# VojtaHavlicek/AlphaZero-Piskvorky

Measured on AMD Instinct MI355X. Metric: mcts_node_expansions_per_sec, higher is better.
Workload: dtype f32; 1 GPU; 15x15 / 5-in-a-row self-play, 1024 concurrent games per GPU, 400 sims/move (BASELINE.json configs[3] per-GPU shard), GomokuNet random-init weights, numpy-compatible RNG tapes; board=15, win_length=5, sims_per_move=400, games_per_gpu=1024, engines_per_gpu=4, search_kernel=lock-step (k_trunk, k_fc, k_step per evaluation batch), parallelism=games sharded x1

## Files before the change

alphazero-piskvorky_amd/_capi.py:

```python
import ctypes as C
import os
import subprocess

import numpy as np

_HERE = os.path.dirname(os.path.abspath(__file__))
LIB_PATH = os.environ.get("AZ_ENGINE_LIB") or os.path.join(_HERE, "libaz_engine.so")

STATE_DICT_ORDER = [
    "conv1.weight", "conv1.bias", "conv2.weight", "conv2.bias", "conv3.weight", "conv3.bias",
    "policy_conv.weight", "policy_conv.bias", "policy_fc.weight", "policy_fc.bias",
    "value_conv.weight", "value_conv.bias", "value_fc1.weight", "value_fc1.bias",
    "value_fc2.weight", "value_fc2.bias",
]

AZ_EVAL_NET, AZ_EVAL_SYNTHETIC = 0, 1
AZ_RES_NONE, AZ_RES_X, AZ_RES_O, AZ_RES_DRAW = 0, 1, 2, 3
AZ_AUG_NONE, AZ_AUG_REFERENCE4, AZ_AUG_DIHEDRAL8 = 1, 4, 8
AZ_MODEL_PLAIN, AZ_MODEL_RESNET = 0, 1
AZ_TRUNK_F32, AZ_TRUNK_BF16X3, AZ_TRUNK_F16X2 = 0, 1, 2
AZ_MAX_SIMULATIONS, AZ_DEEP_MAX_SIMULATIONS = 1024, 65534
REUSE_MAX_SIMULATIONS = 1023

EXPORTS = [
    "az_create", "az_create_deep", "az_destroy", "az_last_error", "az_load_weights", "az_load_weights_resnet", "az_net_eval", "az_search", "az_search_batch", "az_search_callback", "az_selfplay",
    "az_selfplay_begin", "az_selfplay_step", "az_selfplay_end", "az_selfplay_games", "az_selfplay_records", "az_selfplay_clear", "az_record_bytes", "az_selfplay_pack", "az_examples_from_packed",
    "az_examples_gather", "az_arena", "az_rules_replay", "az_rng_selfplay_tape", "az_rng_uniforms", "az_set_profiling", "az_set_subtree_reuse", "az_get_counters", "az_get_lanes", "az_get_persistent", "az_set_virtual_loss", "az_set_eval_cache",
    "az_set_trunk_mode", "az_get_trunk_mode", "az_set_leaf_symmetry", "az_emul_split",
    "az_set_start_positions", "az_get_start_positions",
    "az_set_resign", "az_get_resign", "az_selfplay_values", "az_selfplay_pack_values", "az_selfplay_resign_info",
    "az_resign_mix", "az_resign_exempt",
    "az_set_playout_cap", "az_get_playout_cap", "az_playout_cap_full", "az_selfplay_sims", "az_selfplay_export_count",
    "az_set_forced_playouts", "az_get_forced_playouts", "az_forced_prune",
    "az_set_selection", "az_get_selection", "az_selection_tables",
    "az_set_candidates", "az_get_candidates", "az_candidate_mask",
    "az_set_gumbel", "az_get_gumbel", "az_gumbel_schedule", "az_gumbel_target", "az_gumbel_vmix", "az_rng_selfplay_tape_gumbel",
    "az_set_external_evaluator", "az_get_external_evaluator", "az_ext_capacity", "az_ext_stats",
    "az_set_solver", "az_get_solver", "az_last_proof", "az_selfplay_proofs", "az_solver_counts", "az_solver_stops",
    "az_set_win_rule", "az_get_win_rule", "az_rules_winner",
    "az_set_threat_search", "az_get_threat_search", "az_threat_batch", "az_threat_solve", "az_selfplay_threats", "az_threat_stats",
    "az_set_rng", "az_get_rng", "az_rng_philox4x32", "az_rng_log", "az_rng_exp", "az_rng_philox_tape", "az_rng_philox_tape_device",
    "az_set_delta_eval", "az_get_delta_eval", "az_delta_max_tiles", "az_delta_stats", "az_net_eval_delta", "az_delta_lists",
    "az_dist_unique_id", "az_dist_init", "az_dist_rank", "az_dist_world", "az_dist_counts", "az_dist_gather_records",
    "az_dist_allreduce_sum", "az_dist_broadcast",
]
AZ_DIST_ID_BYTES = 128


class AzError(RuntimeError):
    pass


class az_config(C.Structure):
    _fields_ = [("board_size", C.c_int32), ("win_length", C.c_int32), ("num_simulations", C.c_int32),
                ("slots", C.c_int32), ("c_puct", C.c_double), ("dirichlet_alpha", C.c_double),
                ("dirichlet_weight", C.c_double), ("eval_kind", C.c_int32), ("device", C.c_int32),
                ("log_table", C.POINTER(C.c_float)), ("model", C.c_int32), ("engines", C.c_int32)]


class az_selfplay_args(C.Structure):
    _fields_ = [("seed0", C.c_uint64), ("num_games", C.c_int32), ("max_plies", C.c_int32),
                ("temperature_table", C.POINTER(C.c_double)), ("noise_tape", C.POINTER(C.c_double)),
                ("u_tape", C.POINTER(C.c_double)), ("tape_stride", C.c_int64)]


class az_counters(C.Structure):
    _fields_ = [("games", C.c_int64), ("plies", C.c_int64), ("records", C.c_int64), ("simulations", C.c_int64),
                ("expansions", C.c_int64), ("root_evals", C.c_int64), ("terminal_hits", C.c_int64),
                ("depth_sum", C.c_int64), ("steps", C.c_int64), ("seconds", C.c_double), ("nn_seconds", C.c_double),
                ("trunk_seconds", C.c_double), ("trunk_launches", C.c_int64), ("trunk_boards", C.c_int64),
                ("step_seconds", C.c_double), ("duplicate_leaves", C.c_int64), ("cache_lookups", C.c_int64),
                ("cache_hits", C.c_int64), ("tape_wait_seconds", C.c_double), ("tape_threads", C.c_int64),
                ("host_cpus", C.c_int64)]

    def as_dict(self):
        return {k: getattr(self, k) for k, _ in self._fields_}


class az_arena_args(C.Structure):
    _fields_ = [("seed0", C.c_uint64), ("num_games", C.c_int32), ("temperature_table", C.POINTER(C.c_double)),
                ("u_tape", C.POINTER(C.c_double))]


class az_arena_result(C.Structure):
    _fields_ = [("wins", C.c_int32), ("losses", C.c_int32), ("draws", C.c_int32), ("total", C.c_int32),
                ("win_rate", C.c_double)]


_EVAL_BATCH_FN = C.CFUNCTYPE(C.c_int, C.c_void_p, C.c_int, C.c_int)


class az_ext_evaluator(C.Structure):
    _fields_ = [("planes_dev", C.c_void_p), ("policy_dev", C.c_void_p), ("value_dev", C.c_void_p),
                ("capacity", C.c_int32), ("fn", _EVAL_BATCH_FN), ("user", C.c_void_p)]

# ... 62 lines not shown
            L.az_selfplay_export_count.argtypes = [C.c_void_p, C.POINTER(C.c_int64)]
        if hasattr(L, "az_set_forced_playouts"):
            L.az_set_forced_playouts.argtypes = [C.c_void_p, C.c_double, C.c_int]
            L.az_get_forced_playouts.argtypes = [C.c_void_p, C.POINTER(C.c_double), C.POINTER(C.c_int)]
            L.az_forced_prune.argtypes = [C.c_double, C.c_double, C.c_int, C.c_void_p, C.c_void_p, C.c_void_p, C.c_void_p]
            L.az_forced_prune.restype = C.c_int64
        if hasattr(L, "az_set_selection"):
            L.az_set_selection.argtypes = [C.c_void_p, C.c_int] + [C.c_double] * 4
            L.az_get_selection.argtypes = [C.c_void_p, C.POINTER(C.c_int)] + [C.POINTER(C.c_double)] * 4
            L.az_selection_tables.argtypes = [C.c_double, C.c_double, C.c_double, C.c_int, C.c_void_p, C.c_void_p]
        if hasattr(L, "az_set_candidates"):
            L.az_set_candidates.argtypes = [C.c_void_p, C.c_int]
            L.az_get_candidates.argtypes = [C.c_void_p, C.POINTER(C.c_int)]
            L.az_candidate_mask.argtypes = [C.c_int, C.c_void_p, C.c_int, C.c_void_p]
        if hasattr(L, "az_set_gumbel"):
            L.az_set_gumbel.argtypes = [C.c_void_p, C.c_int, C.c_double, C.c_double]
            L.az_get_gumbel.argtypes = [C.c_void_p, C.POINTER(C.c_int), C.POINTER(C.c_double), C.POINTER(C.c_double)]
            L.az_gumbel_schedule.argtypes = [C.c_int, C.c_int, C.c_void_p]
            L.az_gumbel_target.argtypes = [C.c_int, C.c_void_p, C.c_void_p, C.c_void_p, C.c_void_p, C.c_void_p, C.c_float, C.c_double,
                                           C.c_double, C.c_void_p, C.POINTER(C.c_int32)]
            L.az_gumbel_vmix.argtypes = [C.c_int, C.c_void_p, C.c_void_p, C.c_void_p, C.c_float]
            L.az_gumbel_vmix.restype = C.c_double
            L.az_rng_selfplay_tape_gumbel.argtypes = [C.c_uint64, C.c_int, C.c_int, C.c_void_p, C.c_void_p]
        if hasattr(L, "az_set_external_evaluator"):
            L.az_set_external_evaluator.argtypes = [C.c_void_p, C.POINTER(az_ext_evaluator)]
            L.az_get_external_evaluator.argtypes = [C.c_void_p]
            L.az_ext_capacity.argtypes = [C.c_void_p]
            L.az_ext_stats.argtypes = [C.c_void_p, C.POINTER(C.c_int64), C.POINTER(C.c_int64)]
        if hasattr(L, "az_set_solver"):
            L.az_set_solver.argtypes = [C.c_void_p, C.c_int]
            L.az_get_solver.argtypes = [C.c_void_p]
            L.az_last_proof.argtypes = [C.c_void_p, C.c_int, C.c_void_p, C.c_void_p, C.POINTER(C.c_int32)]
            L.az_solver_stops.argtypes = [C.c_void_p, C.POINTER(C.c_int64)]
            L.az_selfplay_proofs.argtypes = [C.c_void_p, C.c_void_p]
            L.az_solver_counts.argtypes = [C.c_int, C.c_void_p, C.c_void_p, C.c_void_p]
        if hasattr(L, "az_set_win_rule"):
            L.az_set_win_rule.argtypes = [C.c_void_p, C.c_int]
            L.az_get_win_rule.argtypes = [C.c_void_p]
            L.az_rules_winner.argtypes = [C.c_void_p, C.c_int, C.c_int, C.c_int]
        if hasattr(L, "az_set_threat_search"):
            L.az_set_threat_search.argtypes = [C.c_void_p, C.c_int, C.c_int]
            L.az_get_threat_search.argtypes = [C.c_void_p, C.POINTER(C.c_int), C.POINTER(C.c_int)]
            L.az_threat_batch.argtypes = [C.c_void_p, C.c_int, C.c_void_p, C.c_void_p, C.c_int, C.c_int] + [C.c_void_p] * 5
            L.az_threat_solve.argtypes = [C.c_void_p, C.c_int, C.c_int, C.c_int, C.c_int, C.c_int, C.c_int] + [C.c_void_p] * 4
            L.az_selfplay_threats.argtypes = [C.c_void_p, C.c_void_p]
            L.az_threat_stats.argtypes = [C.c_void_p] + [C.POINTER(C.c_int64)] * 5
        if hasattr(L, "az_set_delta_eval"):
            L.az_set_delta_eval.argtypes = [C.c_void_p, C.c_int]
            L.az_get_delta_eval.argtypes = [C.c_void_p]
            L.az_delta_max_tiles.argtypes = [C.c_void_p, C.c_int]
            L.az_delta_stats.argtypes = [C.c_void_p] + [C.POINTER(C.c_int64)] * 4 + [C.c_void_p]
            L.az_net_eval_delta.argtypes = [C.c_void_p, C.c_int, C.c_void_p, C.c_int, C.c_int] + [C.c_void_p] * 7
            L.az_delta_lists.argtypes = [C.c_int, C.c_int] + [C.c_void_p] * 5
        if hasattr(L, "az_set_rng"):
            L.az_set_rng.argtypes = [C.c_void_p, C.c_int]
            L.az_get_rng.argtypes = [C.c_void_p]
            L.az_rng_philox4x32.argtypes = [C.c_void_p, C.c_void_p, C.c_void_p]
            L.az_rng_philox4x32.restype = None
            L.az_rng_log.argtypes = L.az_rng_exp.argtypes = [C.c_double]
            L.az_rng_log.restype = L.az_rng_exp.restype = C.c_double
            L.az_rng_philox_tape.argtypes = [C.c_uint64, C.c_int, C.c_double, C.c_int, C.c_int, C.c_void_p, C.c_void_p]
            L.az_rng_philox_tape_device.argtypes = [C.c_void_p, C.c_uint64, C.c_int, C.c_double, C.c_int, C.c_int, C.c_void_p, C.c_void_p]
        _LIB = L
    return _LIB


def _p(a):
    return None if a is None else a.ctypes.data_as(C.c_void_p)


def _dp(a):
    return None if a is None else a.ctypes.data_as(C.POINTER(C.c_double))


def rng_selfplay_tape(seed, n, alpha=0.3, max_plies=0):
    nn = n * n
    plies = max_plies if 0 < max_plies < nn else nn
    total = sum(nn - m for m in range(plies))
    noise = np.zeros(total, np.float64)
    u = np.zeros(nn, np.float64)
    rc = lib().az_rng_selfplay_tape(int(seed), n, float(alpha), int(max_plies), _p(noise), _p(u))
    if rc:
        raise AzError(f"az_rng_selfplay_tape failed ({rc})")
    return noise, u[:plies]


def dist_unique_id():
    buf = C.create_string_buffer(AZ_DIST_ID_BYTES)
    rc = lib().az_dist_unique_id(buf)
    if rc:
        raise AzError(f"az_dist_unique_id failed ({rc}): {lib().az_last_error(None).decode()}")
    return buf.raw


def rng_uniforms(seed, count):
    u = np.zeros(count, np.float64)
    rc = lib().az_rng_uniforms(int(seed), int(count), _p(u))
    if rc:
        raise AzError(f"az_rng_uniforms failed ({rc})")
    return u


def resign_mix(key):
    return int(lib().az_resign_mix(int(key) & 0xFFFFFFFF))


# ... 845 lines not shown
```

alphazero-piskvorky_amd/csrc/az_delta.h:

```cpp
#pragma once
#include "az_net.h"

constexpr int DELTA_MAX_CHANGED = 8;
constexpr int DELTA_TILES_DEFAULT = 12;
constexpr int DELTA_CNT = 4 + 16;

template <int N>
struct DeltaGeo : NetGeo<N> {
    typedef NetGeo<N> B;
    static constexpr int IMG = 96 * B::CS;
    static constexpr int STRIDE = IMG + B::FROW;
    static constexpr int MAXM = ((B::nn + 15) / 16) * 16;
    static constexpr int C3 = 4;
};

__host__ __device__ inline int delta_dist(int n, int pr, int pc, const unsigned char *changed, int nch)
{
    int best = 255;
    for (int i = 0; i < nch; i++) {
        const int cr = changed[i] / n, cc = changed[i] - cr * n;
        const int dr = pr - 1 - cr < 0 ? cr - (pr - 1) : pr - 1 - cr, dc = pc - 1 - cc < 0 ? cc - (pc - 1) : pc - 1 - cc;
        const int dd = dr > dc ? dr : dc;
        best = dd < best ? dd : best;
    }
    return best;
}
__host__ __device__ inline bool delta_member(int n, int list, int pr, int pc, int dist)
{
    const bool inb = pr >= 1 && pr <= n && pc >= 1 && pc <= n;
    return list < 3 ? (inb && dist <= list + 1) : dist <= list;
}
template <int N>
struct DeltaLists {
    typedef DeltaGeo<N> G;
    unsigned short wpos[3][G::MAXM], cell[3][G::MAXM];
    unsigned short halo[2][G::PP];
    int cnt[5];
    __host__ __device__ int tiles(int l) const { return (cnt[l] + 15) >> 4; }
    __host__ __device__ void put(int list, int at, int pr, int pc)
    {
        const unsigned short pos = (unsigned short)(pr * G::PW + pc);
        if (list < 3) { wpos[list][at] = pos; cell[list][at] = (unsigned short)((pr - 1) * N + (pc - 1)); }
        else halo[list - 3][at] = pos;
    }
    __host__ __device__ void junk(int list, int i)
    {
        const int c = cnt[list], at = c + i;
        if (c > 0 && at < tiles(list) * 16) { wpos[list][at] = wpos[list][c - 1]; cell[list][at] = 0xFFFF; }
    }
};
template <int N>
__host__ __device__ inline void delta_lists_serial(const unsigned char *changed, int nch, DeltaLists<N> &L)
{
    typedef DeltaGeo<N> G;
    for (int l = 0; l < 5; l++) L.cnt[l] = 0;
    for (int p = 0; p < G::PP; p++) {
        const int pr = p / G::PW, pc = p - pr * G::PW;
        const int dist = delta_dist(N, pr, pc, changed, nch);
        for (int l = 0; l < 5; l++)
            if (delta_member(N, l, pr, pc, dist)) L.put(l, L.cnt[l]++, pr, pc);
    }
    for (int l = 0; l < 3; l++)
        for (int i = 0; i < 16; i++) L.junk(l, i);
}

#ifdef __HIPCC__
template <class G>
__device__ __forceinline__ void delta_heads(const NetWeights &w, float *__restrict__ frow, const float *out3, const float *hdq_lds,
                                            const unsigned short *cellof, int ncell, int wave, int lane)
{
    if (wave * 32 >= ncell) return;
    const int half = (lane >> 2) & 1;
    const int m = wave * 32 + (lane >> 3) * 4 + (lane & 3);
    float hb[4];
#pragma unroll
    for (int i = 0; i < 4; i++) hb[i] = (half * 4 + i) < 6 ? w.hdb[half * 4 + i] : 0.0f;
    const float4 *ap = reinterpret_cast<const float4 *>(hdq_lds) + (lane & 7);
    const float4 *bp = reinterpret_cast<const float4 *>(out3 + (m < ncell ? m : 0) * OUT3_CM_STRIDE);
    f32x4 acc = f32x4{0.f, 0.f, 0.f, 0.f};
#pragma unroll
    for (int k4 = 0; k4 < 32; k4++) {
        const float4 a = ap[k4 * 8], b = bp[k4];
        acc = __builtin_amdgcn_mfma_f32_4x4x1f32(a.x, b.x, acc, 0, 0, 0);
        acc = __builtin_amdgcn_mfma_f32_4x4x1f32(a.y, b.y, acc, 0, 0, 0);
        acc = __builtin_amdgcn_mfma_f32_4x4x1f32(a.z, b.z, acc, 0, 0, 0);
        acc = __builtin_amdgcn_mfma_f32_4x4x1f32(a.w, b.w, acc, 0, 0, 0);
    }
    if (m < ncell) {
        const int cell = cellof[m];
        if (cell != 0xFFFF) {
#pragma unroll
            for (int i = 0; i < 4; i++) {
                const int j = half * 4 + i;
                if (j < 6) {
                    float v = acc[i] + hb[i];
                    frow[j * G::nn + cell] = v > 0.0f ? v : 0.0f;
                }
            }
        }
    }
}

template <int N>
__global__ __launch_bounds__(NetGeo<N>::NW * 64) void k_trunk_base(DevState d, NetWeights w, int net_id, float *__restrict__ base,
                                                                    unsigned long long *cnt)
{
    typedef FusedGeo<N> G;
    typedef DeltaGeo<N> DG;
    static_assert(G::G == 1, "one board per workgroup");
    __shared__ __attribute__((aligned(16))) float lds[G::LDSF];
    __shared__ __attribute__((aligned(16))) float hdq_lds[1024];
    __shared__ unsigned short wpos[G::MR];
    __shared__ unsigned short cellof[G::MR];
    const int b = blockIdx.x, par = blockIdx.y;
    if (d.s_status[b] != SLOT_ACTIVE || d.s_net[b] != net_id) return;
    const int tid = threadIdx.x, lane = tid & 63;
    const int wave = __builtin_amdgcn_readfirstlane(tid >> 6);
    const float2 hq = reinterpret_cast<const float2 *>(w.hdq)[tid];
    bool e_me = false, e_op = false;
    int e_pos = G::PW + 1;
    if (tid < G::nn) {
        const int r = tid / N, c = tid - r * N;
        e_pos = (r + 1) * G::PW + (c + 1);
        const u64 *bd = d.board + (size_t)b * 8;
        const bool x = (bd[tid >> 6] >> (tid & 63)) & 1ull, o = (bd[4 + (tid >> 6)] >> (tid & 63)) & 1ull;
        const bool me_is_x = (d.s_player[b] == 1) != (par == 1);
        e_me = me_is_x ? x : o;
        e_op = me_is_x ? o : x;
    }
    reinterpret_cast<float2 *>(hdq_lds)[tid] = hq;
    if (tid < G::MR) {
        if constexpr (BorderSkip<G>::value) { wpos[tid] = G::map.pos[tid]; cellof[tid] = G::map.cell[tid]; }
        else {
            const int t = tid >> 4, c = tid & 15;
            wpos[tid] = (unsigned short)((t + 1) * G::PW + (c + 1));
            cellof[tid] = (unsigned short)(c < N ? t * N + c : 0xFFFF);
        }
    }
    {
        float4 *z = reinterpret_cast<float4 *>(lds);
        for (int i = tid; i < (96 * G::CS) / 4; i += G::NW * 64) z[i] = float4{0.f, 0.f, 0.f, 0.f};
    }
    __syncthreads();
    float *inA = lds, *inB = lds + 32 * G::CS;
    if (e_me) inB[e_pos] = 1.0f;
    if (e_op) inB[G::CS + e_pos] = 1.0f;
    __syncthreads();
    conv_layer<G, 4, 32, CONV_OUT_PACKED>(inB, inA, w.c1, w.c1b, wpos, cellof, wave, lane);
    __syncthreads();
    for (int i = tid; i < 3 * G::CS; i += G::NW * 64) inB[i] = 0.0f;
    __syncthreads();
    conv_layer<G, 32, 64, CONV_OUT_PACKED>(inA, inB, w.c2, w.c2b, wpos, cellof, wave, lane);
    __syncthreads();
    float *row = base + ((size_t)b * 2 + par) * DG::STRIDE;
    {
        const float4 *s = reinterpret_cast<const float4 *>(lds);
        float4 *g = reinterpret_cast<float4 *>(row);
        for (int i = tid; i < DG::IMG / 4; i += G::NW * 64) g[i] = s[i];
    }
    conv_layer<G, 64, 128, CONV_OUT3_CM>(inB, lds, w.c3, w.c3b, wpos, cellof, wave, lane);
    __syncthreads();
    trunk_heads<G>(d, w, net_id, row + DG::IMG - (size_t)b * G::FROW, lds, hdq_lds, cellof, b, wave, lane);
    if (tid == 0 && par == 0) cnt[(size_t)b * DELTA_CNT + 3] += 2ull;
}

template <int N>
__global__ __launch_bounds__(NetGeo<N>::NW * 64) void k_trunk_delta(DevState d, NetWeights w, int net_id, float *__restrict__ feat,
                                                                     const float *__restrict__ base, unsigned char *done,
                                                                     unsigned long long *cnt, int max_tiles)
{
    typedef DeltaGeo<N> G;
    constexpr int NT = G::NW * 64;
    static_assert(G::G == 1 && NT >= G::PP && NT == 512, "one board per workgroup, one thread per padded position");
    static_assert(G::C3 * 16 * OUT3_CM_STRIDE <= 32 * G::CS, "a chunk's conv3 image fits the dead conv1 image");
    static_assert(G::STRIDE % 4 == 0, "16-byte rows");
    __shared__ __attribute__((aligned(16))) float lds[G::IMG];
    __shared__ __attribute__((aligned(16))) float planes[4 * G::CS];
    __shared__ __attribute__((aligned(16))) float hdq_lds[1024];
    __shared__ DeltaLists<N> L;
    __shared__ unsigned char changed[DELTA_MAX_CHANGED];
    __shared__ unsigned char s_dist[G::PP];
    __shared__ int s_nch;
    __shared__ int s_wc[5][5];
    const int b = blockIdx.x;
    if (b >= d.B) return;
    const int tid = threadIdx.x, lane = tid & 63;
    const int wave = __builtin_amdgcn_readfirstlane(tid >> 6);
    {
        const int kind = d.leaf_kind[b];
        if (!((kind == LEAF_ROOT || kind == LEAF_EXPAND) && d.s_status[b] == SLOT_ACTIVE && d.s_net[b] == net_id)) {
            if (tid == 0) done[b] = 1;
            return;
        }
    }
    const float2 hq = reinterpret_cast<const float2 *>(w.hdq)[tid];
    const u64 *lf = d.leaf + (size_t)b * 8, *bd = d.board + (size_t)b * 8;
    const int last = d.leaf_last[b];
    int stones = 0;
#pragma unroll
    for (int i = 0; i < 8; i++) stones += __popcll(lf[i]) - __popcll(bd[i]);
    const int par = stones & 1;
    bool e_me = false, e_op = false, e_last = false;
    int e_pos = G::PW + 1;
    if (tid == 0) s_nch = 0;
    for (int i = tid; i < 4 * G::CS; i += NT) planes[i] = 0.0f;
    reinterpret_cast<float2 *>(hdq_lds)[tid] = hq;
    __syncthreads();
    if (tid < G::nn) {
        const int r = tid / N, c = tid - r * N;
        e_pos = (r + 1) * G::PW + (c + 1);
        e_me = (lf[tid >> 6] >> (tid & 63)) & 1ull;
        e_op = (lf[4 + (tid >> 6)] >> (tid & 63)) & 1ull;
        e_last = last == tid;
        const bool x = (bd[tid >> 6] >> (tid & 63)) & 1ull, o = (bd[4 + (tid >> 6)] >> (tid & 63)) & 1ull;
        const bool me_is_x = (d.s_player[b] == 1) != (par == 1);
        if (e_me != (me_is_x ? x : o) || e_op != (me_is_x ? o : x) || e_last) {
            const int k = atomicAdd(&s_nch, 1);
            if (k < DELTA_MAX_CHANGED) changed[k] = (unsigned char)tid;
        }
        if (e_me) planes[e_pos] = 1.0f;
        if (e_op) planes[G::CS + e_pos] = 1.0f;
        if (e_last) planes[2 * G::CS + e_pos] = 1.0f;
    }
    __syncthreads();
    const int nch = s_nch;
    if (nch > DELTA_MAX_CHANGED) {
        if (tid == 0) { done[b] = 0; cnt[(size_t)b * DELTA_CNT + 1] += 1ull; }
        return;
    }
    int dist = 255, pr = 0, pc = 0;
    u64 bal[5] = {0, 0, 0, 0, 0};
    if (wave < 5) {
        const bool in_img = tid < G::PP;
        if (in_img) {
            pr = tid / G::PW; pc = tid - pr * G::PW;
            dist = delta_dist(N, pr, pc, changed, nch);
            s_dist[tid] = (unsigned char)dist;
        }
#pragma unroll
        for (int l = 0; l < 5; l++) {
            bal[l] = __ballot(in_img && delta_member(N, l, pr, pc, dist));
            if (lane == 0) s_wc[wave][l] = __popcll(bal[l]);
        }
    }
    __syncthreads();
    if (wave < 5 && tid < G::PP) {
#pragma unroll
        for (int l = 0; l < 5; l++) {
            if (!((bal[l] >> lane) & 1ull)) continue;
            int at = __popcll(bal[l] & ((1ull << lane) - 1ull));
            for (int v = 0; v < wave; v++) at += s_wc[v][l];
            L.put(l, at, pr, pc);
        }
    }
    if (tid < 5) L.cnt[tid] = s_wc[0][tid] + s_wc[1][tid] + s_wc[2][tid] + s_wc[3][tid] + s_wc[4][tid];
    __syncthreads();
    const int t1 = L.tiles(0), t2 = L.tiles(1), t3 = L.tiles(2);
    if (t3 > max_tiles) {
        if (tid == 0) { done[b] = 0; cnt[(size_t)b * DELTA_CNT + 1] += 1ull; }
        return;
    }
    if (tid < 48) L.junk(tid >> 4, tid & 15);
    if (tid == 0) {
        done[b] = (unsigned char)(1 + t3);
        cnt[(size_t)b * DELTA_CNT + 0] += 1ull;
        cnt[(size_t)b * DELTA_CNT + 2] += (unsigned long long)t3;
        cnt[(size_t)b * DELTA_CNT + 4 + t3] += 1ull;
    }
    float *inA = lds, *inB = lds + 32 * G::CS;
    const float *brow = base + ((size_t)b * 2 + par) * G::STRIDE;
    {
        const float4 *g4 = reinterpret_cast<const float4 *>(brow);
        float4 *l4 = reinterpret_cast<float4 *>(lds);
        const int n3 = L.cnt[3], n4 = L.cnt[4];
        for (int i = tid; i < 8 * n3; i += NT) {
            const int pl = i / n3, at = pl * G::CS + L.halo[0][i - pl * n3];
            l4[at] = g4[at];
        }
        for (int i = tid; i < 16 * n4; i += NT) {
            const int pl = i / n4, at = (8 + pl) * G::CS + L.halo[1][i - pl * n4];
            l4[at] = g4[at];
        }
        const float *bf = brow + G::IMG;
        float *frow = feat + (size_t)b * G::FROW;
        for (int i = tid; i < 6 * G::nn; i += NT) {
            const int p = i % G::nn, r = p / N, c = p - r * N;
            if (s_dist[(r + 1) * G::PW + (c + 1)] > 3) frow[i] = bf[i];
        }
    }
    __syncthreads();
    for (int t0 = 0; t0 < t1; t0 += 4)
        conv_layer<G, 4, 32, CONV_OUT_PACKED, 4>(planes, inA, w.c1, w.c1b, L.wpos[0], L.cell[0], wave, lane, t0, t1 - t0 < 4 ? t1 - t0 : 4);
    __syncthreads();
    for (int t0 = 0; t0 < t2;) {
        const int c = t2 - t0;
        if (c > 2) { conv_layer<G, 32, 64, CONV_OUT_PACKED, 4>(inA, inB, w.c2, w.c2b, L.wpos[1], L.cell[1], wave, lane, t0, c < 4 ? c : 4); t0 += 4; }
        else { conv_layer<G, 32, 64, CONV_OUT_PACKED, 2>(inA, inB, w.c2, w.c2b, L.wpos[1], L.cell[1], wave, lane, t0, c); t0 += 2; }
    }
    __syncthreads();
    float *frow = feat + (size_t)b * G::FROW;
    for (int t0 = 0; t0 < t3; t0 += G::C3) {
        const int c = t3 - t0 < G::C3 ? t3 - t0 : G::C3;
        float *o3 = lds - t0 * 16 * OUT3_CM_STRIDE;
        if (c == 4) conv_layer<G, 64, 128, CONV_OUT3_CM, 4>(inB, o3, w.c3, w.c3b, L.wpos[2], L.cell[2], wave, lane, t0, 4);
        else if (c == 3) conv_layer<G, 64, 128, CONV_OUT3_CM, 3>(inB, o3, w.c3, w.c3b, L.wpos[2], L.cell[2], wave, lane, t0, 3);
        else if (c == 2) conv_layer<G, 64, 128, CONV_OUT3_CM, 2>(inB, o3, w.c3, w.c3b, L.wpos[2], L.cell[2], wave, lane, t0, 2);
        else conv_layer<G, 64, 128, CONV_OUT3_CM, 1>(inB, o3, w.c3, w.c3b, L.wpos[2], L.cell[2], wave, lane, t0, 1);
        __syncthreads();
        delta_heads<G>(w, frow, lds, hdq_lds, L.cell[2] + t0 * 16, c * 16, wave, lane);
        __syncthreads();
    }
}

template <int N>
__global__ __launch_bounds__(NetGeo<N>::NW * 64) void k_trunk_rest(DevState d, NetWeights w, int net_id, float *__restrict__ feat,
                                                                    const unsigned char *done)
{
    typedef FusedGeo<N> G;
    static_assert(G::G == 1, "one board per workgroup");
    __shared__ __attribute__((aligned(16))) float lds[G::LDSF];
    __shared__ __attribute__((aligned(16))) float hdq_lds[1024];
    __shared__ unsigned short wpos[G::MR];
    __shared__ unsigned short cellof[G::MR];
    __shared__ int any_active;
    const int grp = blockIdx.x;
    if (grp >= d.B || done[grp]) return;
    trunk_group<N>(d, w, net_id, feat, nullptr, grp, lds, hdq_lds, wpos, cellof, &any_active, threadIdx.x);
}
#endif
```

alphazero-piskvorky_amd/csrc/az_engine.hip:

```cpp
#include <hip/hip_runtime.h>
#include <dlfcn.h>
#include <sched.h>

#include <algorithm>
#include <atomic>
#include <chrono>
#include <condition_variable>
#include <cmath>
#include <cstdarg>
#include <cstdio>
#include <cstdlib>
#include <cstring>
#include <mutex>
#include <string>
#include <thread>
#include <vector>

#define AZ_ENGINE_TU 1
#include "../../include/az_engine.h"
#include "az_launch.h"

#include "az_host.h"

static thread_local std::string g_create_error;
// ... 2399 lines not shown
{
    if (!e || !stops) return AZ_ERR_INVALID;
    *stops = e->solver_stops;
    return AZ_OK;
}

extern "C" int az_set_delta_eval(az_engine *e, int on)
{
    if (!e) return AZ_ERR_INVALID;
    if (e->run.open) return fail(e, AZ_ERR_STATE, "az_set_delta_eval: an episode is open");
    e->delta_on = on != 0;
    return AZ_OK;
}

extern "C" int az_get_delta_eval(const az_engine *e) { return e ? (e->delta_on ? 1 : 0) : AZ_ERR_INVALID; }

extern "C" int az_delta_max_tiles(az_engine *e, int tiles)
{
    if (!e) return AZ_ERR_INVALID;
    if (tiles == 0) return e->delta_tiles;
    if (e->run.open) return fail(e, AZ_ERR_STATE, "az_delta_max_tiles: an episode is open");
    if (tiles < 1 || tiles > 15) return fail(e, AZ_ERR_INVALID, "az_delta_max_tiles: 1 .. 15 conv3 tiles, 0 asks");
    e->delta_tiles = tiles;
    return tiles;
}

extern "C" int az_delta_stats(const az_engine *e, int64_t *delta, int64_t *full, int64_t *tiles, int64_t *base, int64_t *by_tiles)
{
    if (!e) return AZ_ERR_INVALID;
    if (delta) *delta = e->delta_stats[0];
    if (full) *full = e->delta_stats[1];
    if (tiles) *tiles = e->delta_stats[2];
    if (base) *base = e->delta_stats[3];
    if (by_tiles) for (int t = 0; t < 16; t++) by_tiles[t] = e->delta_stats[4 + t];
    return AZ_OK;
}

extern "C" int az_delta_lists(int n, int count, const uint8_t *changed, uint16_t *wpos, uint16_t *cell, uint16_t *halo, int32_t *cnt)
{
    if (n != 15 || count < 0 || count > DELTA_MAX_CHANGED || (count && !changed) || !wpos || !cell || !halo || !cnt) return AZ_ERR_INVALID;
    for (int i = 0; i < count; i++) if (changed[i] >= 15 * 15) return AZ_ERR_INVALID;
    static DeltaLists<15> L;
    static std::mutex m;
    std::lock_guard<std::mutex> lock(m);
    memset(&L, 0xEE, sizeof L);
    delta_lists_serial<15>(changed, count, L);
    memcpy(wpos, L.wpos, sizeof L.wpos);
    memcpy(cell, L.cell, sizeof L.cell);
    memcpy(halo, L.halo, sizeof L.halo);
    for (int l = 0; l < 5; l++) cnt[l] = L.cnt[l];
    return AZ_OK;
}

extern "C" int az_net_eval_delta(az_engine *e, int slot, const uint8_t *root, int root_player, int count, const uint8_t *boards,
                                 const uint8_t *players, const int16_t *lasts, float *logits, float *policy, float *value, int32_t *path)
{
    if (!e || slot < 0 || slot > 1 || count < 0 || !root || !boards || !players || !lasts || (root_player != 1 && root_player != 2))
        return fail(e, AZ_ERR_INVALID, "az_net_eval_delta: bad argument");
    if (!e->net[slot].loaded) return fail(e, AZ_ERR_NO_WEIGHTS, "weights slot %d not loaded", slot);
    if (e->run.open) return fail(e, AZ_ERR_STATE, "az_net_eval_delta: a self-play episode is open on this engine");
    if (!e->ops->trunk_delta || e->cfg.model != AZ_MODEL_PLAIN || e->cfg.eval_kind != AZ_EVAL_NET)
        return fail(e, AZ_ERR_INVALID, "az_net_eval_delta: no delta evaluation for this board size or net");
    DEVICE_GUARD(e);
    int rc = ensure_delta_buffers(e);
    if (rc) return rc;
    const Lane &L = e->lanes[0];
    const DeltaRoot dr{root, root_player, path};
    return eval_positions(e, "az_net_eval_delta", slot, count, boards, players, lasts, logits, policy, value, &dr, [&](LaunchCtx &lc, int) {
        lc.delta_base = (float *)L.delta_base.p;
        lc.delta_done = (unsigned char *)L.delta_done.p;
        lc.delta_cnt = (unsigned long long *)L.delta_cnt.p;
        lc.delta_tiles = e->delta_tiles;
        e->ops->trunk_base(lc, slot);
        e->ops->trunk_delta(lc, slot);
    });
}

extern "C" int az_selfplay_proofs(az_engine *e, int8_t *roots)
{
    if (!e || !e->have_episode) return fail(e, AZ_ERR_STATE, "no episode has been run");
    if (!roots) return fail(e, AZ_ERR_INVALID, "az_selfplay_proofs: null buffer");
    if (!e->episode_solver || !e->rec_proof.p) return fail(e, AZ_ERR_STATE, "az_selfplay_proofs: the episode ran without the solver");
    DEVICE_GUARD(e);
    return read_record_array(e, e->rec_proof, roots);
}

extern "C" int az_solver_counts(int count, const int32_t *visits, const int8_t *status, int32_t *out)
{
    if (count < 1 || !visits || !status || !out) return AZ_ERR_INVALID;
    bool any_win = false, survivor = false;
    for (int c = 0; c < count; c++) {
        if (visits[c] < 0 || status[c] < 0 || status[c] > 3) return AZ_ERR_INVALID;
        any_win = any_win || status[c] == PROOF_WIN;
        survivor = survivor || (status[c] != PROOF_LOSS && visits[c] > 0);
    }
    for (int c = 0; c < count; c++) out[c] = solver_keeps(status[c], any_win, survivor) ? visits[c] : 0;
    return AZ_OK;
}

static int check_position(az_engine *e, const char *who, const uint8_t *bd, int player, int last, int *stones)
{
    const int nn = e->nn;
    if (player != 1 && player != 2) return fail(e, AZ_ERR_INVALID, "%s: player %d", who, player);
    int st = 0;
    for (int j = 0; j < nn; j++) {
        if (bd[j] > 2) return fail(e, AZ_ERR_INVALID, "%s: cell value %d", who, bd[j]);
// ... 992 lines not shown
```

alphazero-piskvorky_amd/csrc/az_kernels.hip:

```cpp
#include <hip/hip_runtime.h>
#include "az_launch.h"

#ifndef AZ_N
#error "compile with -DAZ_N=<board size>"
#endif
#define AZ_CAT2(a, b) a##b
#define AZ_CAT(a, b) AZ_CAT2(a, b)

namespace {
constexpr int N = AZ_N;

void trunk(const LaunchCtx &c, int net_id)
{
    if (c.model == 1) {
        typedef ResGeo<N> G;
        dim3 gt((c.dv.B + G::G - 1) / G::G), bt(G::NW * 64);
        if (c.emul == EMUL_BF16X3) hipLaunchKernelGGL((k_trunk_res_emul<N, EMUL_BF16X3>), gt, dim3(ResGeoEmul<N>::NW * 64), 0, c.stream, c.dv, c.rw[net_id], net_id, c.feat);
        else if (c.emul == EMUL_F16X2) hipLaunchKernelGGL((k_trunk_res_emul<N, EMUL_F16X2>), gt, dim3(ResGeoEmul<N>::NW * 64), 0, c.stream, c.dv, c.rw[net_id], net_id, c.feat);
        else hipLaunchKernelGGL(k_trunk_res<N>, gt, bt, 0, c.stream, c.dv, c.rw[net_id], net_id, c.feat);
    } else {
        typedef NetGeo<N> G;
        dim3 gt((c.dv.B + G::G - 1) / G::G), bt(G::NW * 64);
        if (c.emul == EMUL_BF16X3) hipLaunchKernelGGL((k_trunk_emul<N, EMUL_BF16X3>), gt, bt, 0, c.stream, c.dv, c.w[net_id], net_id, c.feat, c.dbg);
        else if (c.emul == EMUL_F16X2) hipLaunchKernelGGL((k_trunk_emul<N, EMUL_F16X2>), gt, bt, 0, c.stream, c.dv, c.w[net_id], net_id, c.feat, c.dbg);
// ... 226 lines not shown
    int slots = 0;
    for (int l = 0; l < bl.K; l++) slots += bl.lane[l].B;
    return slots;
}

void set_positions(hipStream_t stream, const BatchLanes &bl, const unsigned char *cells, const unsigned char *players, const short *lasts)
{
    dim3 g((batch_slots(bl) + 3) / 4), b(256);
    hipLaunchKernelGGL(k_set_positions<N>, g, b, 0, stream, bl, cells, players, lasts);
}

void gather_roots(hipStream_t stream, const BatchLanes &bl, const DevState &d, const unsigned char *cells, int *visits, double *W, float *prior, float *pi, int *action)
{
    dim3 g((batch_slots(bl) + 3) / 4), b(256);
    hipLaunchKernelGGL(k_gather_roots<N>, g, b, 0, stream, bl, d.R, d.S, cells, (const float *)d.rec_pi,
                       (const short *)d.rec_action, visits, W, prior, pi, action);
}

void build_positions(hipStream_t stream, int count, const unsigned char *cells, const unsigned char *players, const short *lasts, StartPos *table)
{
    dim3 g((count + 3) / 4), b(256);
    hipLaunchKernelGGL(k_build_positions<N>, g, b, 0, stream, count, cells, players, lasts, table);
}

void ext_gather(const LaunchCtx &c, int net, int item_base, int first, int capacity, float *planes, int *map, int *count)
{
    hipLaunchKernelGGL(k_ext_gather<N>, dim3(1), dim3(EXT_GATHER_THREADS), 0, c.stream, c.dv, net, item_base, first, capacity, planes, map, count);
}

void ext_scatter(const LaunchCtx &c, int item_base, int count, const int *map, const float *policy, const float *value)
{
    dim3 g((count + 3) / 4), b(256);
    hipLaunchKernelGGL(k_ext_scatter<N>, g, b, 0, c.stream, c.dv, item_base, count, map, policy, value);
}

void threat(const LaunchCtx &c)
{
    hipLaunchKernelGGL(k_threat<N>, dim3(c.d.B), dim3(64), 0, c.stream, c.d);
}

constexpr bool HAS_DELTA = N == 15;

void trunk_base(const LaunchCtx &c, int net_id)
{
    if constexpr (HAS_DELTA)
        hipLaunchKernelGGL(k_trunk_base<N>, dim3(c.d.B, 2), dim3(NetGeo<N>::NW * 64), 0, c.stream, c.d, c.w[net_id], net_id, c.delta_base, c.delta_cnt);
}

void trunk_delta(const LaunchCtx &c, int net_id)
{
    if constexpr (HAS_DELTA) {
        const dim3 g(c.dv.B), b(NetGeo<N>::NW * 64);
        hipLaunchKernelGGL(k_trunk_delta<N>, g, b, 0, c.stream, c.dv, c.w[net_id], net_id, c.feat, (const float *)c.delta_base, c.delta_done,
                           c.delta_cnt, c.delta_tiles);
        hipLaunchKernelGGL(k_trunk_rest<N>, g, b, 0, c.stream, c.dv, c.w[net_id], net_id, c.feat, (const unsigned char *)c.delta_done);
    }
}

template <bool ON>
long long delta_floats() { if constexpr (ON) return 2ll * DeltaGeo<N>::STRIDE; else return 0; }
}

const SizeOps *AZ_CAT(az_size_ops_, AZ_N)()
{
    static const SizeOps ops = {trunk, trunk_split, split_scratch_floats, fc, step, step_vl, root_cache, search_prepare, search, move, eval_tail_l,
                                set_positions, gather_roots, build_positions, ext_gather, ext_scatter, threat,
                                HAS_DELTA ? trunk_base : nullptr, HAS_DELTA ? trunk_delta : nullptr, delta_floats<HAS_DELTA>()};
    return &ops;
}
```

include/az_engine.h:

```cpp
#ifndef AZ_ENGINE_H
#define AZ_ENGINE_H

#include <stdint.h>

#ifdef __cplusplus
extern "C" {
#endif

typedef struct az_engine az_engine;

typedef enum {
    AZ_OK = 0,
    AZ_ERR_INVALID = -1,
    AZ_ERR_NO_DEVICE = -2,
    AZ_ERR_HIP = -3,
    AZ_ERR_ILLEGAL_MOVE = -4,
    AZ_ERR_NO_WEIGHTS = -5,
    AZ_ERR_STATE = -6
} az_status;

enum { AZ_EVAL_NET = 0, AZ_EVAL_SYNTHETIC = 1 };
enum { AZ_RES_NONE = 0, AZ_RES_X = 1, AZ_RES_O = 2, AZ_RES_DRAW = 3 };
enum { AZ_AUG_REFERENCE4 = 4, AZ_AUG_DIHEDRAL8 = 8, AZ_AUG_NONE = 1 };
enum { AZ_TRUNK_F32 = 0, AZ_TRUNK_BF16X3 = 1, AZ_TRUNK_F16X2 = 2 };
// ... 111 lines not shown
int az_dist_rank(const az_engine *e);
int az_dist_world(const az_engine *e);
int az_dist_counts(az_engine *e, int64_t *counts);
int az_dist_gather_records(az_engine *e, int dst, void *packed_dev);
int az_dist_allreduce_sum(az_engine *e, int64_t *values, int n);
int az_dist_broadcast(az_engine *e, void *buf_dev, int64_t bytes, int root);

int az_examples_from_packed(az_engine *e, const void *packed_dev, int64_t records, int aug,
                            float *states_dev, float *pis_dev, float *z_dev);

int az_examples_gather(az_engine *e, const void *packed_dev, const int64_t *idx_dev, const int32_t *sym_dev,
                       int count, int reference_pi, float *states_dev, float *pis_dev, float *z_dev);

typedef struct {
    uint64_t seed0;
    int32_t num_games;
    const double *temperature_table;
    const double *u_tape;
} az_arena_args;
typedef struct { int32_t wins, losses, draws, total; double win_rate; } az_arena_result;
int az_arena(az_engine *e, const az_arena_args *args, az_arena_result *out, int32_t *results, int16_t *actions,
             int32_t *nply);

int az_rules_replay(az_engine *e, int games, int max_len, const int16_t *actions, uint8_t *term_before, uint8_t *boards,
                    int32_t *players, int32_t *results, int32_t *first_illegal);

int az_rng_selfplay_tape(uint64_t seed, int board_size, double alpha, int max_plies, double *noise, double *u);
int az_rng_uniforms(uint64_t seed, int count, double *u);
int az_rng_selfplay_tape_gumbel(uint64_t seed, int board_size, int max_plies, double *noise, double *u);

enum { AZ_RNG_NUMPY = 0, AZ_RNG_PHILOX = 1 };
enum { AZ_TAPE_DIRICHLET = 0, AZ_TAPE_GUMBEL = 1 };
#define AZ_RNG_PHILOX_ATTEMPTS 64
int az_set_rng(az_engine *e, int mode);
int az_get_rng(const az_engine *e);
void az_rng_philox4x32(const uint32_t ctr[4], const uint32_t key[2], uint32_t out[4]);
double az_rng_log(double x);
double az_rng_exp(double x);
int az_rng_philox_tape(uint64_t seed, int board_size, double alpha, int max_plies, int kind, double *noise, double *u);
int az_rng_philox_tape_device(az_engine *e, uint64_t seed0, int games, double alpha, int max_plies, int kind, double *noise_out,
                              double *u_out);

int az_set_subtree_reuse(az_engine *e, int on);

int az_set_virtual_loss(az_engine *e, int leaves);

int az_set_eval_cache(az_engine *e, int64_t entries);

int az_set_delta_eval(az_engine *e, int on);
int az_get_delta_eval(const az_engine *e);
int az_delta_max_tiles(az_engine *e, int tiles);
int az_delta_stats(const az_engine *e, int64_t *delta, int64_t *full, int64_t *tiles, int64_t *base, int64_t *by_tiles);
int az_delta_lists(int n, int count, const uint8_t *changed, uint16_t *wpos, uint16_t *cell, uint16_t *halo, int32_t *cnt);
int az_net_eval_delta(az_engine *e, int slot, const uint8_t *root, int root_player, int count, const uint8_t *boards,
                      const uint8_t *players, const int16_t *lasts, float *logits, float *policy, float *value, int32_t *path);

int az_set_leaf_symmetry(az_engine *e, int on);

int az_set_start_positions(az_engine *e, int count, const uint8_t *boards ,
                           const uint8_t *players, const int16_t *lasts, int64_t first);
int az_get_start_positions(const az_engine *e);

enum { AZ_RULE_FREESTYLE = 0, AZ_RULE_EXACT = 1 };
int az_set_win_rule(az_engine *e, int rule);
int az_get_win_rule(const az_engine *e);
int az_rules_winner(const uint8_t *board, int n, int k, int rule);

uint32_t az_resign_mix(uint32_t x);
int az_resign_exempt(uint32_t key, int playout_permille);
int az_set_resign(az_engine *e, double threshold, int min_ply, int playout_permille);
int az_get_resign(const az_engine *e, double *threshold, int *min_ply, int *playout_permille);
int az_selfplay_values(az_engine *e, float *values);
int az_selfplay_pack_values(az_engine *e, float *values_dev);
int az_selfplay_resign_info(az_engine *e, int32_t *cross_ply, uint8_t *exempt);

int az_playout_cap_full(uint32_t key, int ply, int full_permille);
int az_set_playout_cap(az_engine *e, int fast_sims, int full_permille, int export_full_only);
int az_get_playout_cap(const az_engine *e, int *fast_sims, int *full_permille, int *export_full_only);
int az_selfplay_sims(az_engine *e, int32_t *sims);
int az_selfplay_export_count(az_engine *e, int64_t *records);

int az_set_forced_playouts(az_engine *e, double k, int prune);
int az_get_forced_playouts(const az_engine *e, double *k, int *prune);
int64_t az_forced_prune(double k, double c_puct, int count, const int32_t *visits, const double *W, const float *prior, int32_t *out);

int az_set_selection(az_engine *e, int on, double fpu, double fpu_root, double cpuct_base, double cpuct_factor);
int az_get_selection(const az_engine *e, int *on, double *fpu, double *fpu_root, double *cpuct_base, double *cpuct_factor);
int az_selection_tables(double c_puct, double cpuct_base, double cpuct_factor, int S, double *cpuct, double *mass);

int az_set_candidates(az_engine *e, int radius);
int az_get_candidates(const az_engine *e, int *radius);
int az_candidate_mask(int n, const uint8_t *board, int radius, uint8_t *mask);

int az_set_gumbel(az_engine *e, int m, double c_visit, double c_scale);
int az_get_gumbel(const az_engine *e, int *m, double *c_visit, double *c_scale);
int az_gumbel_schedule(int k, int S, int32_t *out);
int az_gumbel_target(int count, const float *logits, const double *g, const int32_t *visits, const double *W, const float *prior,
                     float root_value, double c_visit, double c_scale, float *pi, int32_t *action);
double az_gumbel_vmix(int count, const int32_t *visits, const double *W, const float *prior, float root_value);

enum { AZ_PROOF_UNKNOWN = 0, AZ_PROOF_WIN = 1, AZ_PROOF_LOSS = 2, AZ_PROOF_DRAW = 3 };
int az_set_solver(az_engine *e, int on);
int az_get_solver(const az_engine *e);
int az_last_proof(az_engine *e, int capacity, int8_t *edges, int8_t *roots, int32_t *count);
int az_solver_stops(const az_engine *e, int64_t *stops);
int az_selfplay_proofs(az_engine *e, int8_t *roots);
// ... 29 lines not shown
```

Baseline: 5.609 million node-expansions/s.

## Fold full-trunk fallback into delta kernel and prefetch halo loads into registers

The delta trunk kernel no longer exits for boards with too many changed cells or too many tiles. It now builds full lists in place and runs the whole conv trunk itself, which removes the separate k_trunk_rest launch. Halo and feature-row copies from the base buffer are staged through registers, and the conv2 halo stores are deferred until after conv1, so global load latency can overlap with conv1 compute. This costs extra registers per thread and makes full evaluations go through the tiled delta path, which may be slower than the dedicated fused trunk kernel.

```diff
diff --git a/alphazero-piskvorky_amd/_capi.py b/alphazero-piskvorky_amd/_capi.py
--- a/alphazero-piskvorky_amd/_capi.py
+++ b/alphazero-piskvorky_amd/_capi.py
@@ -40,7 +40,7 @@
     "az_set_win_rule", "az_get_win_rule", "az_rules_winner",
     "az_set_threat_search", "az_get_threat_search", "az_threat_batch", "az_threat_solve", "az_selfplay_threats", "az_threat_stats",
     "az_set_rng", "az_get_rng", "az_rng_philox4x32", "az_rng_log", "az_rng_exp", "az_rng_philox_tape", "az_rng_philox_tape_device",
-    "az_set_delta_eval", "az_get_delta_eval", "az_delta_max_tiles", "az_delta_stats", "az_net_eval_delta", "az_delta_lists",
+    "az_set_delta_eval", "az_get_delta_eval", "az_delta_max_tiles", "az_delta_stats", "az_net_eval_delta", "az_delta_lists", "az_delta_lists_full",
     "az_dist_unique_id", "az_dist_init", "az_dist_rank", "az_dist_world", "az_dist_counts", "az_dist_gather_records",
     "az_dist_allreduce_sum", "az_dist_broadcast",
 ]
@@ -209,6 +209,8 @@
             L.az_delta_stats.argtypes = [C.c_void_p] + [C.POINTER(C.c_int64)] * 4 + [C.c_void_p]
             L.az_net_eval_delta.argtypes = [C.c_void_p, C.c_int, C.c_void_p, C.c_int, C.c_int] + [C.c_void_p] * 7
             L.az_delta_lists.argtypes = [C.c_int, C.c_int] + [C.c_void_p] * 5
+        if hasattr(L, "az_delta_lists_full"):
+            L.az_delta_lists_full.argtypes = [C.c_int] + [C.c_void_p] * 4
         if hasattr(L, "az_set_rng"):
             L.az_set_rng.argtypes = [C.c_void_p, C.c_int]
             L.az_get_rng.argtypes = [C.c_void_p]
diff --git a/alphazero-piskvorky_amd/csrc/az_delta.h b/alphazero-piskvorky_amd/csrc/az_delta.h
--- a/alphazero-piskvorky_amd/csrc/az_delta.h
+++ b/alphazero-piskvorky_amd/csrc/az_delta.h
@@ -63,8 +63,33 @@
     for (int l = 0; l < 3; l++)
         for (int i = 0; i < 16; i++) L.junk(l, i);
 }
+template <int N>
+__host__ __device__ inline void delta_full_put(DeltaLists<N> &L, int pr, int pc)
+{
+    if (pr < 1 || pr > N || pc < 1 || pc > N) return;
+    for (int l = 0; l < 3; l++) L.put(l, (pr - 1) * N + (pc - 1), pr, pc);
+}
+template <int N>
+__host__ __device__ inline void delta_full_cnt(DeltaLists<N> &L, int l) { L.cnt[l] = l < 3 ? N * N : 0; }
+template <int N>
+__host__ __device__ inline void delta_lists_full(DeltaLists<N> &L)
+{
+    typedef DeltaGeo<N> G;
+    for (int p = 0; p < G::PP; p++) delta_full_put<N>(L, p / G::PW, p % G::PW);
+    for (int l = 0; l < 5; l++) delta_full_cnt<N>(L, l);
+    for (int l = 0; l < 3; l++)
+        for (int i = 0; i < 16; i++) L.junk(l, i);
+}
 
 #ifdef __HIPCC__
+#ifdef AZ_STAMPS
+#define AZ_DSTAMP(k) do { if (threadIdx.x == 0 && dbg) dbg[(size_t)blockIdx.x * 16 + (k)] = __builtin_amdgcn_s_memtime(); } while (0)
+#define AZ_DSTAMP_VAL(k, v) do { if (threadIdx.x == 0 && dbg) dbg[(size_t)blockIdx.x * 16 + (k)] = (unsigned long long)(v); } while (0)
+#else
+#define AZ_DSTAMP(k) do { } while (0)
+#define AZ_DSTAMP_VAL(k, v) do { } while (0)
+#endif
+
 template <class G>
 __device__ __forceinline__ void delta_heads(const NetWeights &w, float *__restrict__ frow, const float *out3, const float *hdq_lds,
                                             const unsigned short *cellof, int ncell, int wave, int lane)
@@ -99,6 +124,12 @@
             }
         }
     }
+}
+
+template <int K, int E, class F>
+__device__ __forceinline__ void delta_rounds(F &&f)
+{
+    if constexpr (K < E) { f(std::integral_constant<int, K>{}); delta_rounds<K + 1, E>(f); }
 }
 
 template <int N>
@@ -167,7 +198,7 @@
 template <int N>
 __global__ __launch_bounds__(NetGeo<N>::NW * 64) void k_trunk_delta(DevState d, NetWeights w, int net_id, float *__restrict__ feat,
                                                                      const float *__restrict__ base, unsigned char *done,
-                                                                     unsigned long long *cnt, int max_tiles)
+                                                                     unsigned long long *cnt, int max_tiles, unsigned long long *dbg)
 {
     typedef DeltaGeo<N> G;
     constexpr int NT = G::NW * 64;
@@ -179,13 +210,17 @@
     __shared__ __attribute__((aligned(16))) float hdq_lds[1024];
     __shared__ DeltaLists<N> L;
     __shared__ unsigned char changed[DELTA_MAX_CHANGED];
-    __shared__ unsigned char s_dist[G::PP];
     __shared__ int s_nch;
     __shared__ int s_wc[5][5];
     const int b = blockIdx.x;
     if (b >= d.B) return;
     const int tid = threadIdx.x, lane = tid & 63;
     const int wave = __builtin_amdgcn_readfirstlane(tid >> 6);
+    AZ_DSTAMP(0);
+    AZ_DSTAMP_VAL(14, __builtin_amdgcn_s_memrealtime());
+#ifdef AZ_STAMPS
+    for (int k = 1; k < 14; k++) AZ_DSTAMP_VAL(k, 0);
+#endif
     {
         const int kind = d.leaf_kind[b];
         if (!((kind == LEAF_ROOT || kind == LEAF_EXPAND) && d.s_status[b] == SLOT_ACTIVE && d.s_net[b] == net_id)) {
@@ -224,81 +259,115 @@
     }
     __syncthreads();
     const int nch = s_nch;
-    if (nch > DELTA_MAX_CHANGED) {
-        if (tid == 0) { done[b] = 0; cnt[(size_t)b * DELTA_CNT + 1] += 1ull; }
-        return;
-    }
-    int dist = 255, pr = 0, pc = 0;
-    u64 bal[5] = {0, 0, 0, 0, 0};
-    if (wave < 5) {
-        const bool in_img = tid < G::PP;
-        if (in_img) {
-            pr = tid / G::PW; pc = tid - pr * G::PW;
-            dist = delta_dist(N, pr, pc, changed, nch);
-            s_dist[tid] = (unsigned char)dist;
-        }
-#pragma unroll
-        for (int l = 0; l < 5; l++) {
-            bal[l] = __ballot(in_img && delta_member(N, l, pr, pc, dist));
-            if (lane == 0) s_wc[wave][l] = __popcll(bal[l]);
-        }
-    }
-    __syncthreads();
-    if (wave < 5 && tid < G::PP) {
-#pragma unroll
-        for (int l = 0; l < 5; l++) {
-            if (!((bal[l] >> lane) & 1ull)) continue;
-            int at = __popcll(bal[l] & ((1ull << lane) - 1ull));
-            for (int v = 0; v < wave; v++) at += s_wc[v][l];
-            L.put(l, at, pr, pc);
-        }
-    }
-    if (tid < 5) L.cnt[tid] = s_wc[0][tid] + s_wc[1][tid] + s_wc[2][tid] + s_wc[3][tid] + s_wc[4][tid];
-    __syncthreads();
+    bool full = nch > DELTA_MAX_CHANGED;
+    const int pr = tid / G::PW, pc = tid - pr * G::PW;
+    int dist = 255;
+    if (!full) {
+        u64 bal[5] = {0, 0, 0, 0, 0};
+        if (wave < 5) {
+            const bool in_img = tid < G::PP;
+            if (in_img) dist = delta_dist(N, pr, pc, changed, nch);
+#pragma unroll
+            for (int l = 0; l < 5; l++) {
+                bal[l] = __ballot(in_img && delta_member(N, l, pr, pc, dist));
+                if (lane == 0) s_wc[wave][l] = __popcll(bal[l]);
+            }
+        }
+        __syncthreads();
+        if (wave < 5 && tid < G::PP) {
+#pragma unroll
+            for (int l = 0; l < 5; l++) {
+                if (!((bal[l] >> lane) & 1ull)) continue;
+                int at = __popcll(bal[l] & ((1ull << lane) - 1ull));
+                for (int v = 0; v < wave; v++) at += s_wc[v][l];
+                L.put(l, at, pr, pc);
+            }
+        }
+        if (tid < 5) L.cnt[tid] = s_wc[0][tid] + s_wc[1][tid] + s_wc[2][tid] + s_wc[3][tid] + s_wc[4][tid];
+        __syncthreads();
+        full = L.tiles(2) > max_tiles;
+        if (full) __syncthreads();
+    }
+    float *inA = lds, *inB = lds + 32 * G::CS;
+    if (full) {
+        if (tid < G::PP) delta_full_put<N>(L, pr, pc);
+        if (tid < 5) delta_full_cnt<N>(L, tid);
+        float4 *z = reinterpret_cast<float4 *>(lds);
+        for (int i = tid; i < G::IMG / 4; i += NT) z[i] = float4{0.f, 0.f, 0.f, 0.f};
+        __syncthreads();
+    }
     const int t1 = L.tiles(0), t2 = L.tiles(1), t3 = L.tiles(2);
-    if (t3 > max_tiles) {
-        if (tid == 0) { done[b] = 0; cnt[(size_t)b * DELTA_CNT + 1] += 1ull; }
-        return;
-    }
+    AZ_DSTAMP(1);
+    AZ_DSTAMP_VAL(13, t3);
     if (tid < 48) L.junk(tid >> 4, tid & 15);
     if (tid == 0) {
-        done[b] = (unsigned char)(1 + t3);
-        cnt[(size_t)b * DELTA_CNT + 0] += 1ull;
-        cnt[(size_t)b * DELTA_CNT + 2] += (unsigned long long)t3;
-        cnt[(size_t)b * DELTA_CNT + 4 + t3] += 1ull;
-    }
-    float *inA = lds, *inB = lds + 32 * G::CS;
-    const float *brow = base + ((size_t)b * 2 + par) * G::STRIDE;
-    {
-        const float4 *g4 = reinterpret_cast<const float4 *>(brow);
-        float4 *l4 = reinterpret_cast<float4 *>(lds);
-        const int n3 = L.cnt[3], n4 = L.cnt[4];
-        for (int i = tid; i < 8 * n3; i += NT) {
-            const int pl = i / n3, at = pl * G::CS + L.halo[0][i - pl * n3];
-            l4[at] = g4[at];
-        }
-        for (int i = tid; i < 16 * n4; i += NT) {
-            const int pl = i / n4, at = (8 + pl) * G::CS + L.halo[1][i - pl * n4];
-            l4[at] = g4[at];
-        }
+        if (full) { done[b] = 0; cnt[(size_t)b * DELTA_CNT + 1] += 1ull; }
+        else {
+            done[b] = (unsigned char)(1 + t3);
+            cnt[(size_t)b * DELTA_CNT + 0] += 1ull;
+            cnt[(size_t)b * DELTA_CNT + 2] += (unsigned long long)t3;
+            cnt[(size_t)b * DELTA_CNT + 4 + t3] += 1ull;
+        }
+    }
+    constexpr int WR = (G::PP + 63) / 64;
+    static_assert(WR * 64 >= G::PP && G::NW == 8, "the rounds reach the longest list; one conv1 plane and two conv2 planes per wave");
+    f32x4 w1[WR], w2[2][WR];
+    float fr[6];
+    f32x4 *l4 = reinterpret_cast<f32x4 *>(lds);
+    float *frow = feat + (size_t)b * G::FROW;
+    const bool keep = !full && tid < G::PP && delta_member(N, 2, pr, pc, 0) && dist > 3;
+    const int fcell = (pr - 1) * N + (pc - 1);
+    const int n3 = full ? 0 : L.cnt[3], n4 = full ? 0 : L.cnt[4];
+    {
+        const float *brow = base + ((size_t)b * 2 + par) * G::STRIDE;
+        const f32x4 *g4 = reinterpret_cast<const f32x4 *>(brow);
         const float *bf = brow + G::IMG;
-        float *frow = feat + (size_t)b * G::FROW;
-        for (int i = tid; i < 6 * G::nn; i += NT) {
-            const int p = i % G::nn, r = p / N, c = p - r * N;
-            if (s_dist[(r + 1) * G::PW + (c + 1)] > 3) frow[i] = bf[i];
-        }
-    }
-    __syncthreads();
+        delta_rounds<0, WR>([&](auto jc) {
+            constexpr int j = decltype(jc)::value;
+            if (j * 64 + lane < n3) w1[j] = g4[wave * G::CS + L.halo[0][j * 64 + lane]];
+        });
+        delta_rounds<0, WR>([&](auto jc) {
+            constexpr int j = decltype(jc)::value;
+            if (j * 64 + lane < n4) {
+                const int pos = L.halo[1][j * 64 + lane];
+                w2[0][j] = g4[(8 + wave) * G::CS + pos];
+                w2[1][j] = g4[(16 + wave) * G::CS + pos];
+            }
+        });
+        if (keep) {
+#pragma unroll
+            for (int i = 0; i < 6; i++) fr[i] = bf[i * G::nn + fcell];
+        }
+        delta_rounds<0, WR>([&](auto jc) {
+            constexpr int j = decltype(jc)::value;
+            if (j * 64 + lane < n3) l4[wave * G::CS + L.halo[0][j * 64 + lane]] = w1[j];
+        });
+    }
+    __syncthreads();
+    AZ_DSTAMP(2);
     for (int t0 = 0; t0 < t1; t0 += 4)
         conv_layer<G, 4, 32, CONV_OUT_PACKED, 4>(planes, inA, w.c1, w.c1b, L.wpos[0], L.cell[0], wave, lane, t0, t1 - t0 < 4 ? t1 - t0 : 4);
-    __syncthreads();
+    delta_rounds<0, WR>([&](auto jc) {
+        constexpr int j = decltype(jc)::value;
+        if (j * 64 + lane < n4) {
+            const int pos = L.halo[1][j * 64 + lane];
+            l4[(8 + wave) * G::CS + pos] = w2[0][j];
+            l4[(16 + wave) * G::CS + pos] = w2[1][j];
+        }
+    });
+    if (keep) {
+#pragma unroll
+        for (int i = 0; i < 6; i++) frow[i * G::nn + fcell] = fr[i];
+    }
+    __syncthreads();
+    AZ_DSTAMP(3);
     for (int t0 = 0; t0 < t2;) {
         const int c = t2 - t0;
         if (c > 2) { conv_layer<G, 32, 64, CONV_OUT_PACKED, 4>(inA, inB, w.c2, w.c2b, L.wpos[1], L.cell[1], wave, lane, t0, c < 4 ? c : 4); t0 += 4; }
         else { conv_layer<G, 32, 64, CONV_OUT_PACKED, 2>(inA, inB, w.c2, w.c2b, L.wpos[1], L.cell[1], wave, lane, t0, c); t0 += 2; }
     }
     __syncthreads();
-    float *frow = feat + (size_t)b * G::FROW;
+    AZ_DSTAMP(4);
     for (int t0 = 0; t0 < t3; t0 += G::C3) {
         const int c = t3 - t0 < G::C3 ? t3 - t0 : G::C3;
         float *o3 = lds - t0 * 16 * OUT3_CM_STRIDE;
@@ -307,24 +376,11 @@
         else if (c == 2) conv_layer<G, 64, 128, CONV_OUT3_CM, 2>(inB, o3, w.c3, w.c3b, L.wpos[2], L.cell[2], wave, lane, t0, 2);
         else conv_layer<G, 64, 128, CONV_OUT3_CM, 1>(inB, o3, w.c3, w.c3b, L.wpos[2], L.cell[2], wave, lane, t0, 1);
         __syncthreads();
+        AZ_DSTAMP(5 + 2 * (t0 / G::C3));
         delta_heads<G>(w, frow, lds, hdq_lds, L.cell[2] + t0 * 16, c * 16, wave, lane);
         __syncthreads();
-    }
-}
-
-template <int N>
-__global__ __launch_bounds__(NetGeo<N>::NW * 64) void k_trunk_rest(DevState d, NetWeights w, int net_id, float *__restrict__ feat,
-                                                                    const unsigned char *done)
-{
-    typedef FusedGeo<N> G;
-    static_assert(G::G == 1, "one board per workgroup");
-    __shared__ __attribute__((aligned(16))) float lds[G::LDSF];
-    __shared__ __attribute__((aligned(16))) float hdq_lds[1024];
-    __shared__ unsigned short wpos[G::MR];
-    __shared__ unsigned short cellof[G::MR];
-    __shared__ int any_active;
-    const int grp = blockIdx.x;
-    if (grp >= d.B || done[grp]) return;
-    trunk_group<N>(d, w, net_id, feat, nullptr, grp, lds, hdq_lds, wpos, cellof, &any_active, threadIdx.x);
+        AZ_DSTAMP(6 + 2 * (t0 / G::C3));
+        AZ_DSTAMP_VAL(15, __builtin_amdgcn_s_memrealtime());
+    }
 }
 #endif
diff --git a/alphazero-piskvorky_amd/csrc/az_engine.hip b/alphazero-piskvorky_amd/csrc/az_engine.hip
--- a/alphazero-piskvorky_amd/csrc/az_engine.hip
+++ b/alphazero-piskvorky_amd/csrc/az_engine.hip
@@ -2475,6 +2475,21 @@
     return AZ_OK;
 }
 
+extern "C" int az_delta_lists_full(int n, uint16_t *wpos, uint16_t *cell, uint16_t *halo, int32_t *cnt)
+{
+    if (n != 15 || !wpos || !cell || !halo || !cnt) return AZ_ERR_INVALID;
+    static DeltaLists<15> L;
+    static std::mutex m;
+    std::lock_guard<std::mutex> lock(m);
+    memset(&L, 0xEE, sizeof L);
+    delta_lists_full<15>(L);
+    memcpy(wpos, L.wpos, sizeof L.wpos);
+    memcpy(cell, L.cell, sizeof L.cell);
+    memcpy(halo, L.halo, sizeof L.halo);
+    for (int l = 0; l < 5; l++) cnt[l] = L.cnt[l];
+    return AZ_OK;
+}
+
 extern "C" int az_net_eval_delta(az_engine *e, int slot, const uint8_t *root, int root_player, int count, const uint8_t *boards,
                                  const uint8_t *players, const int16_t *lasts, float *logits, float *policy, float *value, int32_t *path)
 {
diff --git a/alphazero-piskvorky_amd/csrc/az_kernels.hip b/alphazero-piskvorky_amd/csrc/az_kernels.hip
--- a/alphazero-piskvorky_amd/csrc/az_kernels.hip
+++ b/alphazero-piskvorky_amd/csrc/az_kernels.hip
@@ -302,8 +302,7 @@
     if constexpr (HAS_DELTA) {
         const dim3 g(c.dv.B), b(NetGeo<N>::NW * 64);
         hipLaunchKernelGGL(k_trunk_delta<N>, g, b, 0, c.stream, c.dv, c.w[net_id], net_id, c.feat, (const float *)c.delta_base, c.delta_done,
-                           c.delta_cnt, c.delta_tiles);
-        hipLaunchKernelGGL(k_trunk_rest<N>, g, b, 0, c.stream, c.dv, c.w[net_id], net_id, c.feat, (const unsigned char *)c.delta_done);
+                           c.delta_cnt, c.delta_tiles, c.dbg);
     }
 }
 
diff --git a/include/az_engine.h b/include/az_engine.h
--- a/include/az_engine.h
+++ b/include/az_engine.h
@@ -187,6 +187,7 @@
 int az_delta_max_tiles(az_engine *e, int tiles);
 int az_delta_stats(const az_engine *e, int64_t *delta, int64_t *full, int64_t *tiles, int64_t *base, int64_t *by_tiles);
 int az_delta_lists(int n, int count, const uint8_t *changed, uint16_t *wpos, uint16_t *cell, uint16_t *halo, int32_t *cnt);
+int az_delta_lists_full(int n, uint16_t *wpos, uint16_t *cell, uint16_t *halo, int32_t *cnt);
 int az_net_eval_delta(az_engine *e, int slot, const uint8_t *root, int root_player, int count, const uint8_t *boards,
                       const uint8_t *players, const int16_t *lasts, float *logits, float *policy, float *value, int32_t *path);
 
```

Measured after the change: 6.597 million node-expansions/s, median of 6. +17.6%, better.
